# dluvizon/scene-aware-3d-multi-human

Hardware: AMD Instinct MI355X
Metric: optimizer iterations/sec (N humans x T frames) (higher is better)
Workload: dtype f32 (the two dense LBS contractions as split-16-bit MFMA operands -- three products of (hi, lo) fp16 / bf16 terms, fp32 accumulate; everything else plain fp32)

## Files before the change

include/mhmocap_hip.h:

```cpp
#ifndef MHMOCAP_HIP_H
#define MHMOCAP_HIP_H

#include <stddef.h>
#include <stdint.h>

#ifdef __cplusplus
extern "C" {
#endif

#define MH_NUM_JOINTS 24
#define MH_NUM_BETAS 10
#define MH_NUM_POSE_BASIS 207
#define MH_NUM_KP 17
#define MH_FEAT_STRIDE 224

typedef enum mh_status {
  MH_OK = 0,
  MH_ERR_INVALID = -1,
  MH_ERR_HIP = -2,
  MH_ERR_NO_DEVICE = -3,
  MH_ERR_UNSUPPORTED = -4
} mh_status;

typedef struct mh_model mh_model;
// ... 142 lines not shown
  const float* gbeta_b;
  const float* gxs_b;
  int B, NB, nbeta;
  long long off_betas;
  long long off_xscale;
} mh_person_sums;
int mh_rmsprop_step_person(float* params, float* grads, float* square_avg, float* momentum_buf, size_t n,
                           float lr, float alpha, float momentum, float eps, const float* log_src,
                           float* log_dst, int nlog, int32_t* poke_dst, int npoke, int32_t poke0,
                           int32_t poke1, const mh_person_sums* person, void* stream);
int mh_rmsprop_step_dev(float* params, const float* grads, float* square_avg, float* momentum_buf,
                        size_t n, float* lr_dev, float gamma, float alpha, float momentum, float eps,
                        void* stream);
int mh_adam_step(float* params, const float* grads, float* exp_avg, float* exp_avg_sq, size_t n,
                 int step, float lr, float beta1, float beta2, float eps, void* stream);

int mh_one_euro_scan(const float* x, float* y, int T, size_t E, float min_cutoff, float beta,
                     float frame_rate, void* stream);

int mh_one_euro_scan_shard(const float* x, float* y, int T, size_t E, float min_cutoff, float beta,
                           float frame_rate, int first_frame, float time_before,
                           const float* xprev_in, const float* dxprev_in, float* dxprev_out,
                           void* stream);

int mh_velocity_term(int T, int N, const float* pT , const float* prev_halo,
                     const float* next_halo, float coef, float* gpT, float* loss_out, void* stream);
size_t mh_filtered_verts_workspace_bytes(int T, size_t E);
int mh_filtered_verts_term(int T, size_t E, const float* verts, const float* verts_filt,
                           const float* prev_v, const float* prev_vf, const float* next_v,
                           const float* next_vf, float coef, float* gverts, float* loss_out,
                           void* ws, void* stream);
int mh_filtered_verts_term_init(int T, size_t E, const float* verts, const float* verts_filt,
                                const float* prev_v, const float* prev_vf, const float* next_v,
                                const float* next_vf, float coef, float* gverts, float* loss_out,
                                void* ws, void* stream);
int mh_filtered_verts_term_init_gated(int T, size_t E, const float* verts, const float* verts_filt,
                                      const float* prev_v, const float* prev_vf, const float* next_v,
                                      const float* next_vf, float coef, float* gverts, float* loss_out,
                                      const int32_t* live_dev, void* ws, void* stream);

int mh_pack_masks(const float* seg , int T, int N, int H, int W,
                  uint32_t* bits , float* area , void* stream);
int mh_erode_bits(const uint32_t* in, uint32_t* out , int T, int H, int W, void* stream);
int mh_stage_gates(const float* pose2d , const float* area , int B, float thr,
                   float min_area, float* pose2d_valid , float* mask_valid , void* stream);

// ... 272 lines not shown
```

scene-aware-3d-multi-human_amd/csrc/mh_optim.hip:

```cpp
#include "mh_common.h"

struct ProjP {
  int B, mode, has_kd;
  float K[9];
  float Kd[5];
  float jw[MH_NKP];
  float thr, w, h, coef;
  const float* joints;
  const float* pose2d;
  float* uv;
  float* gj;
  float* loss;
  int NB;
  const float* local;
  const float* xscale;
  const float* transl;
  float* gtransl;
};

__global__ __launch_bounds__(64) void k_project_loss(ProjP p) {
  const int b = blockIdx.x, j = threadIdx.x;
  float l = 0.f;
  float g3[3] = {0.f, 0.f, 0.f};
  if (j < MH_NKP) {
// ... 297 lines not shown
  return MH_OK;
}

__device__ __forceinline__ float one_euro_step(float xi, int i, float frame_rate, float min_cutoff, float beta, float& ti,
                                               float& tp, float& xp, float& dxp) {
#pragma clang fp contract(off)
  const float two_pi = 6.283185307179586f;
  ti = ti + (float)((double)i / (double)frame_rate);
  const float te = ti - tp;
  float r = two_pi * te;
  const float ad = r / (r + 1.f);
  const float dx = (xi - xp) / te;
  const float dxh = ad * dx + (1.f - ad) * dxp;
  const float cutoff = min_cutoff + beta * fabsf(dxh);
  r = (two_pi * cutoff) * te;
  const float a = r / (r + 1.f);
  const float xh = a * xi + (1.f - a) * xp;
  xp = xh;
  dxp = dxh;
  tp = ti;
  return xh;
}

__global__ void k_one_euro(const float* x, float* y, int T, size_t E, float min_cutoff, float beta, float frame_rate,
                           int i0, float t0, const float* xprev_in, const float* dxprev_in, float* dxprev_out) {
  for (size_t e = blockIdx.x * (size_t)blockDim.x + threadIdx.x; e < E; e += (size_t)gridDim.x * blockDim.x) {
    float xp, dxp, tp, ti;
    int first;
    if (xprev_in) {
      xp = xprev_in[e];
      dxp = dxprev_in[e];
      tp = ti = t0;
      first = 0;
    } else {
      xp = x[e];
      dxp = 0.f;
      tp = ti = 0.f;
      y[e] = xp;
      first = 1;
    }
    int k = first;
    for (; k + 8 <= T; k += 8) {
      float xv[8];
#pragma unroll
      for (int u = 0; u < 8; ++u) xv[u] = x[(size_t)(k + u) * E + e];
#pragma unroll
      for (int u = 0; u < 8; ++u)
        y[(size_t)(k + u) * E + e] = one_euro_step(xv[u], i0 + k + u, frame_rate, min_cutoff, beta, ti, tp, xp, dxp);
    }
    for (; k < T; ++k)
      y[(size_t)k * E + e] = one_euro_step(x[(size_t)k * E + e], i0 + k, frame_rate, min_cutoff, beta, ti, tp, xp, dxp);
    if (dxprev_out) dxprev_out[e] = dxp;
  }
}

static int one_euro_launch(const float* x, float* y, int T, size_t E, float min_cutoff, float beta, float frame_rate,
                           int i0, float t0, const float* xprev_in, const float* dxprev_in, float* dxprev_out,
                           void* stream) {
  MH_CHECK(x && y, "null argument");
  MH_CHECK(T >= 1 && E >= 1, "empty input");
  MH_CHECK((xprev_in == nullptr) == (dxprev_in == nullptr), "state arrays come in pairs");
  MH_CHECK(xprev_in || i0 == 0, "a shard that does not start the sequence needs the incoming state");
  const size_t nb = (E + 255) / 256;
  hipLaunchKernelGGL(k_one_euro, dim3((unsigned)(nb < 4096 ? nb : 4096)), dim3(256), 0, (hipStream_t)stream, x, y, T, E,
                     min_cutoff, beta, frame_rate, i0, t0, xprev_in, dxprev_in, dxprev_out);
  MH_LAUNCH_CHECK();
  return MH_OK;
}

extern "C" int mh_one_euro_scan(const float* x, float* y, int T, size_t E, float min_cutoff, float beta,
                                float frame_rate, void* stream) {
  return one_euro_launch(x, y, T, E, min_cutoff, beta, frame_rate, 0, 0.f, nullptr, nullptr, nullptr, stream);
}

extern "C" int mh_one_euro_scan_shard(const float* x, float* y, int T, size_t E, float min_cutoff, float beta,
                                      float frame_rate, int first_frame, float time_before, const float* xprev_in,
                                      const float* dxprev_in, float* dxprev_out, void* stream) {
  return one_euro_launch(x, y, T, E, min_cutoff, beta, frame_rate, first_frame, time_before, xprev_in, dxprev_in,
                         dxprev_out, stream);
}

__global__ __launch_bounds__(256) void k_velocity(int T, int N, const float* pT, const float* prev, const float* next,
                                                  float coef, float* gpT, float* loss_out) {
  __shared__ float s[256];
  const size_t E = (size_t)N * 3, n = (size_t)T * E;
  float acc = 0.f;
  for (size_t i = threadIdx.x; i < n; i += 256) {
    const size_t t = i / E, e = i % E;
    const float c = pT[i];
    float g = 0.f;
    if (t > 0 || prev) {
      const float d = c - (t > 0 ? pT[i - E] : prev[e]);
      acc += d * d;
      g += 2.f * d;
    }
// ... 246 lines not shown
```

scene-aware-3d-multi-human_amd/mhhip/_lib.py:

```python
import ctypes
import os
import re

import numpy as np

HERE = os.path.dirname(os.path.abspath(__file__))
LIB_PATH = os.environ.get('MHHIP_LIB') or os.path.join(HERE, 'libmhmocap_hip.so')
HEADER = os.path.join(os.path.dirname(os.path.dirname(HERE)), 'include', 'mhmocap_hip.h')

c_float_p = ctypes.POINTER(ctypes.c_float)
c_int_p = ctypes.POINTER(ctypes.c_int32)
vp = ctypes.c_void_p


class MhError(RuntimeError):
    pass


class ModelHost(ctypes.Structure):
    _fields_ = [('num_verts', ctypes.c_int32), ('num_faces', ctypes.c_int32),
                ('v_template', c_float_p), ('shapedirs', c_float_p), ('posedirs', c_float_p),
                ('J_regressor', c_float_p), ('lbs_weights', c_float_p), ('parents', c_int_p),
                ('faces', c_int_p), ('reg_alphapose', c_float_p), ('reg_h36m17', c_float_p),
                ('reg_mupots', c_float_p), ('reg_extra9', c_float_p)]
# ... 54 lines not shown
        L.mh_lbs_backward_ex.argtypes = [vp, ctypes.c_int, ctypes.c_int] + [vp] * 15
        L.mh_joints_regress_backward.argtypes = [vp, ctypes.c_int, ctypes.c_int, vp, ctypes.c_int, vp, vp, vp]
        L.mh_project_joints_loss.argtypes = [ctypes.c_int, vp, c_float_p, c_float_p, vp, ctypes.c_float, ctypes.c_int,
                                             ctypes.c_float, ctypes.c_float, ctypes.c_float, vp, vp, vp, vp]
        L.mh_project_joints_loss_w.argtypes = [ctypes.c_int, vp, c_float_p, c_float_p, c_float_p, vp, ctypes.c_float,
                                               ctypes.c_int, ctypes.c_float, ctypes.c_float, ctypes.c_float, vp, vp, vp, vp]
        L.mh_warmup_project_w.argtypes = [ctypes.c_int, ctypes.c_int, vp, vp, vp, c_float_p, c_float_p, c_float_p, vp,
                                          ctypes.c_float, ctypes.c_float, vp, vp, vp]
        L.mh_lbs_set_mode.argtypes = [ctypes.c_int]
        L.mh_lbs_set_forward_pipeline.argtypes = [ctypes.c_int]
        L.mh_rmsprop_step.argtypes = [vp, vp, vp, vp, ctypes.c_size_t] + [ctypes.c_float] * 4 + [vp]
        L.mh_rmsprop_step_log.argtypes = [vp, vp, vp, vp, ctypes.c_size_t] + [ctypes.c_float] * 4 + [vp, vp, ctypes.c_int, vp]
        L.mh_rmsprop_step_log_poke.argtypes = [vp, vp, vp, vp, ctypes.c_size_t] + [ctypes.c_float] * 4 + [vp, vp, ctypes.c_int, vp,
                                                                                                   ctypes.c_int, ctypes.c_int32, ctypes.c_int32, vp]
        L.mh_rmsprop_step_person.argtypes = [vp, vp, vp, vp, ctypes.c_size_t] + [ctypes.c_float] * 4 + [vp, vp, ctypes.c_int, vp,
                                                                                                 ctypes.c_int, ctypes.c_int32, ctypes.c_int32,
                                                                                                 ctypes.POINTER(PersonSums), vp]
        L.mh_lbs_backward_person_partials.argtypes = [vp, ctypes.c_int, vp, ctypes.POINTER(vp), ctypes.POINTER(vp)]
        L.mh_lbs_person_reduce.argtypes = [vp, ctypes.c_int, ctypes.c_int, vp, vp, vp, vp]
        L.mh_rmsprop_step_dev.argtypes = [vp, vp, vp, vp, ctypes.c_size_t, vp] + [ctypes.c_float] * 4 + [vp]
        L.mh_adam_step.argtypes = [vp, vp, vp, vp, ctypes.c_size_t, ctypes.c_int] + [ctypes.c_float] * 4 + [vp]
        L.mh_one_euro_scan.argtypes = [vp, vp, ctypes.c_int, ctypes.c_size_t] + [ctypes.c_float] * 3 + [vp]
        L.mh_one_euro_scan_shard.argtypes = [vp, vp, ctypes.c_int, ctypes.c_size_t] + [ctypes.c_float] * 3 + [ctypes.c_int, ctypes.c_float, vp, vp, vp, vp]
        L.mh_velocity_term.argtypes = [ctypes.c_int, ctypes.c_int, vp, vp, vp, ctypes.c_float, vp, vp, vp]
        L.mh_filtered_verts_term.argtypes = [ctypes.c_int, ctypes.c_size_t] + [vp] * 6 + [ctypes.c_float, vp, vp, vp, vp]
        L.mh_filtered_verts_term_init.argtypes = [ctypes.c_int, ctypes.c_size_t] + [vp] * 6 + [ctypes.c_float, vp, vp, vp, vp]
        L.mh_filtered_verts_term_init_gated.argtypes = [ctypes.c_int, ctypes.c_size_t] + [vp] * 6 + [ctypes.c_float, vp, vp, vp, vp, vp]
        L.mh_filtered_verts_workspace_bytes.restype = ctypes.c_size_t
        L.mh_filtered_verts_workspace_bytes.argtypes = [ctypes.c_int, ctypes.c_size_t]
        u32p = vp
        L.mh_warmup_project.argtypes = [ctypes.c_int, ctypes.c_int, vp, vp, vp, c_float_p, c_float_p, vp,
                                        ctypes.c_float, ctypes.c_float, vp, vp, vp]
        L.mh_pack_masks.argtypes = [vp] + [ctypes.c_int] * 4 + [u32p, vp, vp]
        L.mh_erode_bits.argtypes = [u32p, u32p] + [ctypes.c_int] * 3 + [vp]
        L.mh_stage_gates.argtypes = [vp, vp, ctypes.c_int, ctypes.c_float, ctypes.c_float, vp, vp, vp]
        L.mh_sil_mask_stats.argtypes = [u32p] + [ctypes.c_int] * 4 + [vp] * 8
        L.mh_sil_mask_stats_cached.argtypes = [u32p] + [ctypes.c_int] * 4 + [vp] * 9
        L.mh_prior_terms.argtypes = [ctypes.c_int] * 3 + [vp] * 6 + [ctypes.c_float] * 2 + [vp] * 6
        L.mh_reduce_sum.argtypes = [vp, ctypes.c_size_t, ctypes.c_float, vp, vp]
        L.mh_reduce_sum_multi.argtypes = [ctypes.c_int, ctypes.POINTER(vp), ctypes.POINTER(ctypes.c_size_t), ctypes.POINTER(vp), vp]
        L.mh_reduce_sum2.argtypes = [vp, vp, ctypes.c_size_t, ctypes.c_float, vp, vp, vp]
        L.mh_lowest_vertex.argtypes = [vp, ctypes.c_int, ctypes.c_int, vp, vp, vp]
        L.mh_contact_knn.argtypes = [vp, ctypes.c_int, vp, ctypes.c_int, ctypes.c_int, vp, vp]
        L.mh_scene_workspace_bytes.restype = ctypes.c_size_t
        L.mh_scene_workspace_bytes.argtypes = [ctypes.c_int] * 3
        L.mh_scene_median.argtypes = [ctypes.c_int] * 3 + [vp] * 8
# ... 140 lines not shown
```

scene-aware-3d-multi-human_amd/mhhip/engine.py:

```python
import ctypes
import pickle

import numpy as np
import torch

from . import _lib
from ._lib import check, ptr

H36M_ROW_ORDER = [6, 5, 4, 1, 2, 3, 16, 15, 14, 11, 12, 13, 8, 10, 0, 7, 9]
REG_ALPHAPOSE, REG_H36M17, REG_MUPOTS, REG_EXTRA9 = 0, 1, 2, 3
NUM_REG_JOINTS = {0: 17, 1: 17, 2: 17, 3: 9}


class _ChStub(object):

    def __setstate__(self, state):
        self.__dict__.update(state if isinstance(state, dict) else {'x': state})

    def __array__(self, dtype=None, copy=None):
        x = self.__dict__.get('x', None)
        if x is None:
            raise ValueError('unsupported chumpy object in the SMPL pickle')
        return np.array(x, dtype=dtype) if copy else np.asarray(x, dtype=dtype)

# ... 275 lines not shown
    check(_lib.lib().mh_rmsprop_step_log_poke(ptr(params), ptr(grads), ptr(sq), ptr(buf), params.numel(), lr, alpha, momentum,
                                              eps, ptr(log_src), ptr(log_dst), nlog, poke_dst.data_ptr(), min(len(poke) - 1, 2),
                                              poke[0], poke[1], _lib.stream_ptr(params.device)))


def adam_step(params, grads, m, v, step, lr, b1=0.5, b2=0.5, eps=1e-6):
    check(_lib.lib().mh_adam_step(ptr(params), ptr(grads), ptr(m), ptr(v), params.numel(), int(step), lr, b1, b2, eps,
                                  _lib.stream_ptr(params.device)))


def one_euro_scan(x, min_cutoff, beta, frame_rate=25.0, out=None):
    x = x.contiguous()
    if out is None:
        y = torch.empty_like(x)
    else:
        assert out.is_contiguous() and out.dtype == x.dtype and out.numel() == x.numel() and out.device == x.device
        y = out.view(x.shape)
    T = x.shape[0]
    check(_lib.lib().mh_one_euro_scan(ptr(x), ptr(y), T, x.numel() // T, float(min_cutoff), float(beta),
                                      float(frame_rate), _lib.stream_ptr(x.device)))
    return y


def one_euro_time_before(first_frame, frame_rate=25.0):
    t = np.float32(0)
    for i in range(1, int(first_frame)):
        t = np.float32(t + np.float32(i / frame_rate))
    return float(t)


def one_euro_scan_shard(x, min_cutoff, beta, first_frame, state_in=None, frame_rate=25.0):
    x = x.contiguous()
    y = torch.empty_like(x)
    T = x.shape[0]
    E = x.numel() // T
    dx_out = torch.empty(E, dtype=torch.float32, device=x.device)
    xp, dxp = (None, None) if state_in is None else state_in
    check(_lib.lib().mh_one_euro_scan_shard(ptr(x), ptr(y), T, E, float(min_cutoff), float(beta), float(frame_rate),
                                            int(first_frame), one_euro_time_before(first_frame, frame_rate),
                                            ptr(xp), ptr(dxp), ptr(dx_out), _lib.stream_ptr(x.device)))
    return y, (y[-1].reshape(-1).contiguous(), dx_out)


def velocity_term(pT, coef, gpT, prev_halo=None, next_halo=None):
    T, N = pT.shape[0], pT.shape[1]
    loss = torch.empty(1, dtype=torch.float32, device=pT.device)
# ... 17 lines not shown
```

scene-aware-3d-multi-human_amd/mhhip/sequence.py:

```python
import ctypes

import numpy as np
import os
import torch

from . import _lib, engine, queues
from ._lib import check, ptr

LOG_KEYS = ['loss_pose24j', 'loss_depth', 'loss_silhouette', 'reg_ref_poses', 'reg_scale', 'reg_contact',
            'reg_foot_sliding', 'reg_vel', 'reg_filter_verts']
COEF_KEYS = ['proj2d', 'depth', 'silhouette', 'reg_velocity', 'reg_verts_filter', 'reg_poses', 'reg_scales',
             'reg_contact', 'reg_foot_sliding']
PEN_DEFAULTS = dict(reg_scene_pen=0.0, scene_pen_margin=0.05, scene_pen_band=0.5, scene_pen_edge=0.25)
PEN_LOG = 12
ORDER_DEFAULTS = dict(reg_order=0.0, order_margin=0.05, order_delta=0.5)
ORDER_LOG = 13


_SHARED_STREAMS = {}


def _shared_stream(device, role):
    key = (torch.device(device).index or 0, role)
    st = _SHARED_STREAMS.get(key)
# ... 59 lines not shown
        self.ws2 = model.backward_workspace(B)
        self.kp_ws = torch.empty(max(1, _lib.lib().mh_keypoint_workspace_bytes(model.handle, B)), dtype=torch.uint8, device=self.dev)
        self.fv_ws = torch.empty(_lib.lib().mh_filtered_verts_workspace_bytes(T, N * self.V * 3), dtype=torch.uint8, device=self.dev)
        self.verts = z(B, self.V, 3)
        self.vposed = z(B, self.V, 3)
        self.gverts = None
        self.kp = z(B, 17, 3)
        self.gj = z(B, 17, 3)
        self.uv = z(B, 17, 2)
        self.loss2d = z(B)
        self.prior_body = z(B)
        self.loss3 = z(3)
        self.vel_loss = z(1)
        self.filt_loss = z(1)
        self.log = z(max_cycles, 16)
        self.tmp_log = self._grads_log[n:]
        self._log_pending = None
        self.scene_pts = None
        self.scene_grid = None
        self.scene_M = 0
        self.scene_zmap = None
        self._scene_dev = None
        self._scene_pending = False
        self.verts_filt = None
        self.pT_filt = None
        self.has_images = False
        self.halo = None
        self.phase = torch.zeros(4, dtype=torch.int32, device=self.dev)
        self._phase_const = [torch.tensor([1, k], dtype=torch.int32, device=self.dev) for k in (0, 1)]
        self._phase_host = [0, 0, 0]
        self._phase_poke = None
        self._filt_gate = False
        self.batch_frames = None
        self.timing = None
        if self._pen:
            self.pen_body = z(B)
            self.pen_acc = torch.zeros(B, dtype=torch.int64, device=self.dev)
        if self._order:
            self.order_body = z(B)
            self.order_acc = torch.zeros(B, 3, dtype=torch.int64, device=self.dev)
            self.order_gate = None

    def enable_timing(self, on=True):
        self.timing = {} if on else None

    def _tic(self, name):
        if self.timing is None:
            return None
# ... 20 lines not shown
    def set_batch_table(self, table):
        if table is None:
            self.batch_frames = None
            return
        n = self.nbatches * self.batch
        if getattr(self, 'batch_frames', None) is None or self.batch_frames.numel() != n:
            self.batch_frames = torch.full((n,), -1, dtype=torch.int32, device=self.dev)
        if isinstance(table, torch.Tensor):
            self.batch_frames.copy_(table.reshape(-1), non_blocking=True)
        else:
            self.batch_frames.copy_(torch.as_tensor(np.ascontiguousarray(table, dtype=np.int32).reshape(-1)))

    def _view(self, buf, i, shape):
        return buf[int(self.offs[i]):int(self.offs[i + 1])].view(*shape)

    def leaf(self, name, buf=None):
        buf = self.params if buf is None else buf
        T, N = self.T, self.N
        i, shape = {'poses_T': (0, (T, N, 3)), 'poses_smpl': (1, (T, N, 72)), 'zmin_lin': (2, (T,)),
                    'zmax_lin': (3, (T,)), 'betas': (4, (N, 10)), 'xscale': (5, (N,))}[name]
        return self._view(buf, i, shape)

    def set_leaves(self, poses_T, poses_smpl, betas, zmin_lin, zmax_lin, xscale=None):
        self.leaf('poses_T').copy_(_dev(poses_T, self.dev).view(self.T, self.N, 3))
        self.leaf('poses_smpl').copy_(_dev(poses_smpl, self.dev).view(self.T, self.N, 72))
        self.leaf('betas').copy_(_dev(betas, self.dev).view(self.N, 10))
        self.leaf('zmin_lin').copy_(_dev(zmin_lin, self.dev).view(self.T))
        self.leaf('zmax_lin').copy_(_dev(zmax_lin, self.dev).view(self.T))
        if xscale is not None:
            self.leaf('xscale').copy_(_dev(xscale, self.dev).view(self.N))
        else:
            self.leaf('xscale').zero_()
        self.sq.zero_()
        self.buf.zero_()

    def stage(self, pose2d, poses_ref, valid, betas_ref, seg_mask=None, depths=None):
        T, N, H, W = self.T, self.N, self.H, self.W
        L = _lib.lib()
        st = _lib.stream_ptr(self.dev)
        if getattr(self, '_graphs', None):
            torch.cuda.current_stream(self.dev).synchronize()
            self._graphs = {}
            self._lane_tests = {}
            self._pickers = {}
        self._scene_dev = None
        self.pose2d = _dev(pose2d, self.dev).view(self.B, 17, 3)
# ... 194 lines not shown
        k = d['ready']
        s = d['sets'][k]
        d['front'], d['ready'] = s, None
        self._phase_poke = (1, k)
        self.scene_pts = s['pts']
        self.scene_grid = s['grid']
        self.scene_M = self.H * self.W
        self._scene_event = s['ev']
        self._scene_pending = True

    def _scene_sel(self):
        d = self._scene_dev
        if d is None or os.environ.get('MHHIP_UNIFORM') == '0':
            return None
        if self.scene_pts is None or any(self.scene_pts is x['pts'] for x in d['sets']):
            return d['sets']
        return None

    def _flush_phase(self):
        if self._phase_poke is not None:
            (live, k), self._phase_poke = self._phase_poke, None
            self.phase[1:3].copy_(self._phase_const[k])
            self._phase_host[1], self._phase_host[2] = live, k

    def enable_filter_gate(self):
        if self.verts_filt is not None or self.pT_filt is not None:
            return self._filt_gate
        self.pT_filt = torch.zeros(self.T, self.N, 3, dtype=torch.float32, device=self.dev)
        self.verts_filt = torch.zeros(self.T, self.N, self.V, 3, dtype=torch.float32, device=self.dev)
        self._filt_gate = True
        return True

    def _filters_live(self):
        if self._filt_gate and not self._phase_host[0]:
            self.phase[0:1].fill_(1)
            self._phase_host[0] = 1

    def main_stream(self):
        return torch.cuda.current_stream(self.dev)

    def stream_ctx(self, stream):
        return torch.cuda.stream(stream)

    def scene_median_rows(self, depths_t, back_t, zmin, zmax, med, msk, stream):
        rows, frames = depths_t.shape
        check(_lib.lib().mh_scene_median_t(frames, 1, rows, ptr(depths_t), ptr(back_t), ptr(zmin), ptr(zmax), ptr(med), ptr(msk),
                                           ptr(self._scene_dev['ws']), stream.cuda_stream))

    def scene_fill_plane(self, val, mask, ksize, stream):
        check(_lib.lib().mh_scene_fill(self.H, self.W, int(ksize), 1, ptr(val), ptr(mask), ptr(self._scene_dev['ws']), stream.cuda_stream))

    def scene_device_image(self, images):
# ... 60 lines not shown
        if regress:
            self._regress(_lib.stream_ptr(self.dev))

    def _regress(self, st):
        check(_lib.lib().mh_joints_regress(self.m.handle, self.joints_reg[0], self.B, ptr(self.verts),
                                           ptr(self.leaf('poses_T')), self.joints_reg[1], ptr(self.kp), st))

    def _halo_forward(self, h, st):
        Bh = int(h['poses'].shape[0])
        if getattr(self, '_halo_verts', None) is None or self._halo_verts.shape[0] != Bh:
            self._halo_verts = torch.empty(Bh, self.V, 3, dtype=torch.float32, device=self.dev)
            self._halo_ws = self.m.workspace(Bh)
        check(_lib.lib().mh_lbs_forward(self.m.handle, Bh, self.N, ptr(self.leaf('betas')), ptr(h['poses']), ptr(self.leaf('xscale')),
                                        ptr(h['transl']), ptr(self._halo_verts), None, None, ptr(self._halo_ws), st))
        k = 0
        h['v_prev'] = h['v_next'] = None
        if h.get('has_prev'):
            h['v_prev'] = self._halo_verts[:self.N]
            k = self.N
        if h.get('has_next'):
            h['v_next'] = self._halo_verts[k:k + self.N]

    def step_local(self, lr, alpha=0.5, momentum=0.9, eps=1e-8):
        self._wait_scene_snapshot()
        self._flush_person()
        self._flush_log()
        self._flush_phase()
        lo = self.shared_lo
        engine.rmsprop_step(self.params[:lo], self.grads[:lo], self.sq[:lo], self.buf[:lo], float(lr), alpha, momentum, eps)

    def step_shared(self, lr, alpha=0.5, momentum=0.9, eps=1e-8):
        lo = self.shared_lo
        engine.rmsprop_step(self.params[lo:], self.grads[lo:], self.sq[lo:], self.buf[lo:], float(lr), alpha, momentum, eps)

    def keypoint_terms(self, st):
        jwp = None if self.joint_w is None else self.joint_w.ctypes.data_as(_lib.c_float_p)
        Kp = self.K.ctypes.data_as(_lib.c_float_p)
        Kdp = None if self.Kd is None else self.Kd.ctypes.data_as(_lib.c_float_p)
        check(_lib.lib().mh_keypoint_terms(self.m.handle, self.B, ptr(self.leaf('poses_T')), Kp, Kdp, jwp, ptr(self.pose2d), self.thr,
                                           float(self.W), float(self.H), float(self.c['proj2d']), ptr(self.kp), ptr(self.uv),
                                           ptr(self.gj), ptr(self.loss2d), ptr(self.ws), ptr(self.ws2), ptr(self.kp_ws), st))
        self._kp_chunk = True

    def _side_stream(self):
        if not hasattr(self, '_side'):
            self._side = _shared_stream(self.dev, 'side')
        return self._side

    def cycle(self, row, use_images=True, raster=None):
        self._flush_person()
        nj = raster is not None and use_images and self.has_images
        self.cycle_begin(join=not nj, raster=raster if (use_images and self.has_images) else None)
        self.cycle_finish(row, use_images, raster)

    def cycle_begin(self, join=True, raster=None):
        self._flush_log()
        if not torch.cuda.is_current_stream_capturing():
            self._flush_phase()
        clear_in_fwd = (not join) and raster is not None and _lib.lib().mh_lbs_get_mode() != 0
        if not clear_in_fwd:
            self._grads_log.zero_()
        main = torch.cuda.current_stream(self.dev)
        side = self._side_stream()
        side.wait_stream(main)
        self.forward(regress=False, raster=raster, clear=self._grads_log if clear_in_fwd else None)
        self._leaf_terms_later = not join
        if join:
            self._leaf_terms(side.cuda_stream)
            main.wait_stream(side)

    def _leaf_terms(self, st):
        L, c = _lib.lib(), self.c
        T, N = self.T, self.N
        g, log = self.grads, self.tmp_log
        pT = self.leaf('poses_T')
        h = self.halo or {}
        if self.has_images:
            check(L.mh_sil_mask_stats_cached(ptr(self.bits), T, N, self.H, self.W, ptr(pT), ptr(self.p2d_valid),
                                             ptr(self.mask_valid), ptr(self.front), ptr(self.sil_apply), ptr(self.sil_D),
                                             ptr(self.sil_S), ptr(self.sil_tag), st))
# ... 9 lines not shown
            self.keypoint_terms(st)
            return
        jwp = None if self.joint_w is None else self.joint_w.ctypes.data_as(_lib.c_float_p)
        Kp = self.K.ctypes.data_as(_lib.c_float_p)
        Kdp = None if self.Kd is None else self.Kd.ctypes.data_as(_lib.c_float_p)
        self._kp_chunk = False
        self._regress(st)
        check(_lib.lib().mh_project_joints_loss_w(self.B, ptr(self.kp), Kp, Kdp, jwp, ptr(self.pose2d), self.thr, 0, float(self.W),
                                                  float(self.H), float(self.c['proj2d']), ptr(self.uv), ptr(self.gj), ptr(self.loss2d), st))

    def cycle_finish(self, row, use_images=True, raster=None, scene_ready=False):
        self._finish_a(use_images, raster, scene_ready=scene_ready)
        self._finish_b(row, use_images, raster)

    def _finish_a(self, use_images=True, raster=None, scene_ready=False):
        L = _lib.lib()
        main = torch.cuda.current_stream(self.dev)
        st = main.cuda_stream
        c = self.c
        T, N, B = self.T, self.N, self.B
        h = self.halo or {}
        sel = self._scene_sel() if scene_ready else None
        scene = self.scene_pts is not None or sel is not None
        filt = self.verts_filt is not None and self.pT_filt is not None
        images = use_images and self.has_images
        if self._pen and self.halo is not None:
            raise ValueError('the scene-penetration term (reg_scene_pen != 0) is not available in a frame-sharded run')
        if self._order and self.halo is not None:
            raise ValueError('the depth-ordering term (reg_order != 0) is not available in a frame-sharded run')
        need_gv = scene or filt or (images and raster is not None) or not self.kp_fused
        log = self.tmp_log
        gv = None
        if need_gv:
            if self.gverts is None:
                self.gverts = torch.empty_like(self.verts)
            gv = self.gverts
        self._gv_cur = gv
        side = self._side_stream()
        side.wait_stream(main)
        s2 = side.cuda_stream

        def side_branch():
            self._regress_project(s2)
            if self._leaf_terms_later:
                self._leaf_terms_later = False
                self._leaf_terms(s2)
            with torch.cuda.stream(side):
                if need_gv and filt and h.get('poses') is not None:
                    self._halo_forward(h, s2)
                if need_gv:
                    if filt:
                        E = N * self.V * 3
                        ev = self._tic('filtered_verts')
                        if self._filt_gate:
                            check(L.mh_filtered_verts_term_init_gated(T, E, ptr(self.verts), ptr(self.verts_filt), ptr(h.get('v_prev')),
                                                                      ptr(h.get('vf_prev')), ptr(h.get('v_next')), ptr(h.get('vf_next')),
                                                                      float(c['reg_verts_filter']), ptr(gv), ptr(log[8:9]),
                                                                      self.phase.data_ptr(), ptr(self.fv_ws), s2))
                        else:
                            check(L.mh_filtered_verts_term_init(T, E, ptr(self.verts), ptr(self.verts_filt), ptr(h.get('v_prev')),
                                                                ptr(h.get('vf_prev')), ptr(h.get('v_next')), ptr(h.get('vf_next')),
                                                                float(c['reg_verts_filter']), ptr(gv), ptr(log[8:9]), ptr(self.fv_ws), s2))
                        self._toc(ev)
                    else:
                        gv.zero_()
                if not self.kp_fused:
                    check(L.mh_joints_regress_backward(self.m.handle, self.joints_reg[0], B, ptr(self.gj), self.joints_reg[1], ptr(gv),
                                                       ptr(self.leaf('poses_T', self.grads)), s2))
                if not hasattr(self, '_ev_gv'):
                    self._ev_gv = torch.cuda.Event()
                self._ev_gv.record(side)
            self._scene_done = False
            sums = [(self.loss2d, log[0:1]), (self.prior_body, log[3:4])]
            if scene and (self._scene_dev is None or scene_ready):
                sums += self._scene_terms(s2, reduce=False, sel=sel)
                self._scene_done = True
            _lib.reduce_sum_multi(sums, s2)
        joined = False
        main_first = images and raster is not None
        if not main_first:
            side_branch()
        if images:
            if raster is not None:
# ... 87 lines not shown
        zmap = self._pen_zmap()
        if zmap is None:
            return False
        check(L.mh_scene_pen_term(self.B, self.V, self.H, self.W, Kp, ptr(self.verts), ptr(zmap), *tail))
        return True

    def _order_term(self, raster, st):
        if not self._order:
            return
        c, log = self.c, self.tmp_log
        check(_lib.lib().mh_order_term(*raster.dims, ptr(raster.ws), ptr(self.bits), ptr(self.ebits), ptr(self.order_gate),
                                       float(c['reg_order']), float(c['order_margin']), float(c['order_delta']),
                                       ptr(self.leaf('poses_T', self.grads)), ptr(self.order_body), None, None, ptr(self.order_acc), st))
        _lib.reduce_sum_multi([(self.order_body, log[ORDER_LOG:ORDER_LOG + 1])], st)

    def _finish_b(self, row, use_images=True, raster=None):
        L = _lib.lib()
        st = _lib.stream_ptr(self.dev)
        T, N, B = self.T, self.N, self.B
        g = self.grads
        gpT, gposes = self.leaf('poses_T', g), self.leaf('poses_smpl', g)
        gbetas, gxs = self.leaf('betas', g), self.leaf('xscale', g)
        pT = self.leaf('poses_T')
        filt = self.verts_filt is not None and self.pT_filt is not None
        gv, log = self._gv_cur, self.tmp_log
        if self.scene_pts is not None and not self._scene_done:
            ev = self._tic('scene_terms')
            if self._scene_pending:
                torch.cuda.current_stream(self.dev).wait_event(self._scene_event)
                self._scene_pending = False
            self._scene_terms(st)
            self._toc(ev)
        ev = self._tic('lbs_backward')
        fin, self._raster_fin = getattr(self, '_raster_fin', None), None
        if getattr(self, '_kp_chunk', False):
            pb, px = (None, None) if self._person_now else (ptr(gbetas), ptr(gxs))
            args = (self.m.handle, B, N, ptr(self.leaf('betas')), ptr(self.leaf('poses_smpl')), ptr(self.vposed),
                    ptr(gv), ptr(gposes), ptr(gpT), pb, px, ptr(self.ws), ptr(self.ws2),
                    ctypes.byref(fin) if fin is not None else None, st)
            check(L.mh_lbs_backward_kp_fin(*args))
        else:
            check(L.mh_lbs_backward(self.m.handle, B, N, ptr(self.leaf('betas')), ptr(self.leaf('poses_smpl')),
                                    ptr(self.leaf('xscale')), ptr(pT), ptr(self.vposed), ptr(gv), ptr(self.gj) if self.kp_fused else None, ptr(gposes),
                                    ptr(gpT), None if self._person_now else ptr(gbetas), None if self._person_now else ptr(gxs),
                                    ptr(self.ws), ptr(self.ws2), st))
        self._toc(ev)
        if row is not None:
            self.log[row].copy_(log)

    def step(self, lr, alpha=0.5, momentum=0.9, eps=1e-8):
        self._wait_scene_snapshot()
        poke, self._phase_poke = self._phase_poke, None
        person = None
        if self._person_pending:
            self._person_pending = False
            person = self._person_sums()
        if self._log_pending is not None or poke is not None or person is not None:
            row, self._log_pending = self._log_pending, None
            engine.rmsprop_step_log(self.params, self.grads, self.sq, self.buf, float(lr), self.tmp_log if row is not None else None,
                                    self.log[row] if row is not None else None, alpha, momentum, eps,
                                    poke_dst=self.phase[1:3] if poke is not None else None, poke=poke, person=person)
            if poke is not None:
                self._phase_host[1], self._phase_host[2] = poke
        else:
            engine.rmsprop_step(self.params, self.grads, self.sq, self.buf, float(lr), alpha, momentum, eps)

    def _person_sums(self):
        gb, gx = ctypes.c_void_p(), ctypes.c_void_p()
        check(_lib.lib().mh_lbs_backward_person_partials(self.m.handle, self.B, ptr(self.ws2), ctypes.byref(gb), ctypes.byref(gx)))
        return _lib.PersonSums(gb.value, gx.value, self.B, self.N, 10, int(self.offs[4]), -1 if self.freeze_xscale else int(self.offs[5]))

    def _flush_person(self):
        if self._person_pending:
            self._person_pending = False
            g = self.grads
            check(_lib.lib().mh_lbs_person_reduce(self.m.handle, self.B, self.N, ptr(self.ws2), ptr(self.leaf('betas', g)),
                                                  ptr(self.leaf('xscale', g)), _lib.stream_ptr(self.dev)))

    def _flush_log(self):
        if self._log_pending is not None:
            row, self._log_pending = self._log_pending, None
            self.log[row].copy_(self.tmp_log)

    def _graph_key(self, raster):
        scene = None
        sel = self._scene_sel()
        if sel is not None:
            scene = ('sel', sel[0]['grid'].data_ptr(), sel[1]['grid'].data_ptr())
        elif self.scene_pts is not None:
            scene = (self.scene_pts.data_ptr(), self.scene_grid.data_ptr(), self.scene_M)
        rast = None if raster is None else (raster.ws.data_ptr(), raster.faces.data_ptr())
        bt = None if getattr(self, 'batch_frames', None) is None else self.batch_frames.data_ptr()
        L = _lib.lib()
        glob = (L.mh_raster_get_deterministic(), L.mh_raster_get_sort_margin(), L.mh_lbs_get_mode(), L.mh_raster_get_path(),
                L.mh_raster_get_winners(), float(L.mh_raster_get_sort_defer()), L.mh_lbs_get_forward_pipeline()) if raster is not None else None
        pen = None
        if self._pen:
            zm = tuple(x['zmap'].data_ptr() for x in sel) if sel is not None else (None if self._pen_zmap() is None else self._pen_zmap().data_ptr())
            pen = (float(self.c['reg_scene_pen']), float(self.c['scene_pen_margin']), float(self.c['scene_pen_band']),
                   float(self.c['scene_pen_edge']), zm)
        hk = None if self.halo is None else (bool(self.halo.get('has_prev')), bool(self.halo.get('has_next')), self.halo.get('poses') is not None)
        key = (rast, scene, self.verts_filt is not None and self.pT_filt is not None, self._filt_gate, hk, bt, glob)
        if pen is not None:
            key = key + (pen,)
        if self._order:
            key = key + (('order', float(self.c['reg_order']), float(self.c['order_margin']), float(self.c['order_delta'])),)
        return key

    def raster_terms(self, znear=1.0, zfar=100.0):
        if getattr(self, '_raster', None) is None:
            from . import raster as _raster
            self._raster = _raster.RasterTerms(self, znear, zfar)
        return self._raster

    def replay(self, key, fn, wait_scene=True):
        if wait_scene and self._scene_pending:
            torch.cuda.current_stream(self.dev).wait_event(self._scene_event)
            self._scene_pending = False
        if not hasattr(self, '_graphs'):
            self._graphs = {}
        if not hasattr(self, '_lane_tests'):
            self._lane_tests = {}
        g = self._graphs.get(key)
        if g is None:
            fn()
# ... 7 lines not shown
            lt = self._lane_tests.get(key) if want else None
            if lt is None and want and key not in self._lane_tests:
                lt = self._lane_tests[key] = queues.LaneTest(queues.plan(self.dev), torch.cuda.current_stream(self.dev).cuda_stream)
                lt.clean = True
            if lt is not None and not lt.done and not getattr(lt, 'recorded', False):
                if self._scene_dev.get('snap_pending') or self._scene_pending:
                    lt.clean = False
                main = torch.cuda.current_stream(self.dev)
                lt.before(main)
                g.replay()
                lt.after(main)
            else:
                if lt is not None and not lt.done and lt.poll() and lt.choice is not None:
                    self._scene_move(queues.plan(self.dev).view(lt.choice))
                g.replay()

    def cycle_graphed(self, row, raster=None, scene_update=False):
        self._flush_person()
        self._person_now = bool(self.defer_person) and os.environ.get('MHHIP_DEFER_PERSON') != '0'
        try:
            key = self._graph_key(raster) + (self._person_now,)
            self._flush_log()
            self._flush_phase()
            if scene_update and queues.enabled():
                self._scene_pick(key)
            if scene_update:
                self.scene_device_mark()
            scene_ready = self._scene_dev is not None

            def body():
                nj = raster is not None and self.has_images
                self.cycle_begin(join=not nj, raster=raster if self.has_images else None)
                self.cycle_finish(None, raster=raster, scene_ready=scene_ready)
            self.replay(('full+scene' if scene_ready else 'full',) + key, body)
            if scene_update:
                self.scene_device_launch()
            self._log_pending = row
            self._person_pending = self._person_now
        finally:
            self._person_now = False

    def step_dev(self, alpha=0.5, momentum=0.9, eps=1e-8, gamma=0.99, lr0=0.01):
        if not hasattr(self, 'lr_dev'):
            self.lr_dev = torch.full((1,), lr0, dtype=torch.float32, device=self.dev)
        self._flush_person()
        self._flush_log()
        self._flush_phase()
        self._wait_scene_snapshot()
        check(_lib.lib().mh_rmsprop_step_dev(ptr(self.params), ptr(self.grads), ptr(self.sq), ptr(self.buf),
                                             self.params.numel(), ptr(self.lr_dev), gamma, alpha, momentum, eps,
                                             _lib.stream_ptr(self.dev)))

    def set_filters(self, pT_filt, verts_filt):
        verts_filt = verts_filt.view(self.T, self.N, self.V, 3)
        if self.pT_filt is None or self.pT_filt.shape != pT_filt.shape:
            self.pT_filt = pT_filt.clone()
        else:
            self.pT_filt.copy_(pT_filt)
        if self.verts_filt is None or self.verts_filt.shape != verts_filt.shape:
            self.verts_filt = verts_filt.clone()
        else:
            self.verts_filt.copy_(verts_filt)
        self._filters_live()

    def update_filters(self, c1=0.01, b1=0.02, c2=0.001, b2=0.5):
        pT = self.leaf('poses_T')
        if self.pT_filt is not None and self.verts_filt is not None and self.pT_filt.numel() == pT.numel():
            engine.one_euro_scan(pT, c1, b1, out=self.pT_filt)
            self.forward(regress=False)
            engine.one_euro_scan(self.verts.view(self.T, -1), c2, b2, out=self.verts_filt)
            self._filters_live()
            return
        pf = engine.one_euro_scan(pT, c1, b1)
        self.forward(regress=False)
        self.set_filters(pf, engine.one_euro_scan(self.verts.view(self.T, -1), c2, b2))

    def one_euro_shard(self, x, min_cutoff, beta, first_frame, state_in=None):
        return engine.one_euro_scan_shard(x, min_cutoff, beta, first_frame, state_in)

    def read_log(self, rows, nbatches_total=None):
        self._flush_log()
        raw = self.log[:rows].cpu().numpy().astype(np.float64)
        nb = float(nbatches_total or self.nbatches)
        out = []
        for r in raw:
            d = {'loss_pose24j': r[0] / nb, 'loss_depth': r[1] / nb, 'loss_silhouette': r[2] / nb,
                 'reg_ref_poses': (r[3] + r[9]) / nb, 'reg_scale': r[10] + r[11], 'reg_contact': r[5] / nb,
                 'reg_foot_sliding': r[6] / nb, 'reg_vel': r[7], 'reg_filter_verts': r[8]}
            if self._pen:
                d['reg_scene_pen'] = r[PEN_LOG]
            if self._order:
                d['reg_order'] = r[ORDER_LOG]
            out.append({k: np.float32(v) for k, v in d.items()})
# ... 2 lines not shown
```

scene-aware-3d-multi-human_amd/mhmocap/optimizer.py:

```python
import os

import numpy as np
import torch
import torch.distributed as dist

from mhhip import _lib, engine
from mhhip.sequence import SequenceEngine, COEF_KEYS
from .smpl import SMPL
from .transforms import get_focal, softplus_np

try:
    from tqdm import tqdm
except Exception:
    tqdm = None


def frames_arg(frames, T):
    idx = np.arange(T) if frames is None else np.asarray(frames).reshape(-1)
    if idx.size == 0 or not np.issubdtype(idx.dtype, np.integer) or idx.min() < 0 or idx.max() >= T:
        raise ValueError('frames must be indices in [0, %d), got %r' % (T, frames))
    return idx.astype(np.int64)


class SMPLOptimizerBase(object):
# ... 471 lines not shown
        lr = 0.01
        e.sq.zero_()
        e.buf.zero_()
        sh.leaves_changed()
        sh.refresh_halo()
        if (self.use_graphs and world == 1 and os.environ.get('MHHIP_UNIFORM') != '0' and hasattr(e, 'enable_filter_gate')):
            if (num_iter > 30 and scene_mode == 'device' and e.has_images and self._backmasks is not None and e._scene_dev is None):
                sh.scene_setup(self._backmasks)
            if any(c % update_filters_every == 0 for c in range(30, num_iter)):
                e.enable_filter_gate()
        deferring = bool(self.use_graphs and world == 1 and hasattr(e, 'defer_person'))
        if deferring:
            defer_before = e.defer_person
            e.defer_person, e.freeze_xscale = True, not self.optim_scale_factor
        cycles = range(num_iter)
        if verbose and tqdm is not None and rank == 0:
            cycles = tqdm(cycles)
        for cycle in cycles:
            if cycle >= 30 and cycle % update_filters_every == 0:
                if world > 1:
                    sh.update_filters(min_cutoff1, beta1, min_cutoff2, beta2)
                else:
                    e.update_filters(min_cutoff1, beta1, min_cutoff2, beta2)
                self.poses_T_filtered = e.pT_filt.view(e.T, self.num_people, 1, 3)
                self.verts_filtered = e.verts_filt
            if tables is not None:
                e.set_batch_table(tables[cycle])
            scene_now = cycle >= 30 and e.has_images and self._backmasks is not None
            dev_scene = scene_now and scene_mode == 'device'
            if dev_scene and e._scene_dev is None:
                sh.scene_setup(self._backmasks)
            if world > 1:
                if dev_scene:
                    sh.scene_update()
                sh.cycle(cycle, raster=raster, graphs=self.use_graphs)
            else:
                sh.cycle(cycle, raster=raster, graphs=self.use_graphs, scene_update=dev_scene)
            if dev_scene:
                e.scene_device_swap()
            if not self.optim_scale_factor:
                e.leaf('xscale', e.grads).zero_()
            sh.step(lr)
            lr *= 0.99
            if check_every and cycle % check_every == 0:
                self.check_replicas()
        if deferring:
            e._flush_person()
            e.defer_person = defer_before
# ... 227 lines not shown
```

Before: 1638.

## Defer one-euro filter update into captured cycle via device-gated fused scan kernel

Instead of running the two one-euro scans and an extra forward pass eagerly whenever the filters are refreshed, the update is recorded as pending. Inside the next cycle it runs as a single gated kernel that filters both vertices and root translations, reusing the vertices the cycle's forward pass just produced. A device control word arms the gate and is cleared afterwards through the optimizer-step poke, so the captured graph stays the same. This removes an extra forward pass and several launches per filter update, at the cost of more complex host state and flush points.

```diff
diff --git a/include/mhmocap_hip.h b/include/mhmocap_hip.h
--- a/include/mhmocap_hip.h
+++ b/include/mhmocap_hip.h
@@ -188,6 +188,9 @@
                            float frame_rate, int first_frame, float time_before,
                            const float* xprev_in, const float* dxprev_in, float* dxprev_out,
                            void* stream);
+
+int mh_one_euro_scan2_gated(const int32_t* ctl, const float* xa, float* ya, size_t Ea, const float* xb,
+                            float* yb, size_t Eb, int T, float frame_rate, void* stream);
 
 int mh_velocity_term(int T, int N, const float* pT , const float* prev_halo,
                      const float* next_halo, float coef, float* gpT, float* loss_out, void* stream);
diff --git a/scene-aware-3d-multi-human_amd/csrc/mh_optim.hip b/scene-aware-3d-multi-human_amd/csrc/mh_optim.hip
--- a/scene-aware-3d-multi-human_amd/csrc/mh_optim.hip
+++ b/scene-aware-3d-multi-human_amd/csrc/mh_optim.hip
@@ -343,9 +343,10 @@
   return xh;
 }
 
-__global__ void k_one_euro(const float* x, float* y, int T, size_t E, float min_cutoff, float beta, float frame_rate,
-                           int i0, float t0, const float* xprev_in, const float* dxprev_in, float* dxprev_out) {
-  for (size_t e = blockIdx.x * (size_t)blockDim.x + threadIdx.x; e < E; e += (size_t)gridDim.x * blockDim.x) {
+__device__ __forceinline__ void one_euro_channels(const float* x, float* y, int T, size_t E, float min_cutoff, float beta,
+                                                  float frame_rate, int i0, float t0, const float* xprev_in,
+                                                  const float* dxprev_in, float* dxprev_out, size_t e0, size_t stride) {
+  for (size_t e = e0; e < E; e += stride) {
     float xp, dxp, tp, ti;
     int first;
     if (xprev_in) {
@@ -375,6 +376,24 @@
   }
 }
 
+__global__ void k_one_euro(const float* x, float* y, int T, size_t E, float min_cutoff, float beta, float frame_rate,
+                           int i0, float t0, const float* xprev_in, const float* dxprev_in, float* dxprev_out) {
+  one_euro_channels(x, y, T, E, min_cutoff, beta, frame_rate, i0, t0, xprev_in, dxprev_in, dxprev_out,
+                    blockIdx.x * (size_t)blockDim.x + threadIdx.x, (size_t)gridDim.x * blockDim.x);
+}
+
+__global__ void k_one_euro2_gated(const int* ctl, const float* xa, float* ya, size_t Ea, unsigned nba, const float* xb,
+                                  float* yb, size_t Eb, int T, float frame_rate) {
+  if (ctl[0] == 0) return;
+  const float* par = (const float*)(ctl + 1);
+  if (blockIdx.x < nba)
+    one_euro_channels(xa, ya, T, Ea, par[0], par[1], frame_rate, 0, 0.f, nullptr, nullptr, nullptr,
+                      blockIdx.x * (size_t)blockDim.x + threadIdx.x, (size_t)nba * blockDim.x);
+  else
+    one_euro_channels(xb, yb, T, Eb, par[2], par[3], frame_rate, 0, 0.f, nullptr, nullptr, nullptr,
+                      (blockIdx.x - nba) * (size_t)blockDim.x + threadIdx.x, (size_t)(gridDim.x - nba) * blockDim.x);
+}
+
 static int one_euro_launch(const float* x, float* y, int T, size_t E, float min_cutoff, float beta, float frame_rate,
                            int i0, float t0, const float* xprev_in, const float* dxprev_in, float* dxprev_out,
                            void* stream) {
@@ -392,6 +411,18 @@
 extern "C" int mh_one_euro_scan(const float* x, float* y, int T, size_t E, float min_cutoff, float beta,
                                 float frame_rate, void* stream) {
   return one_euro_launch(x, y, T, E, min_cutoff, beta, frame_rate, 0, 0.f, nullptr, nullptr, nullptr, stream);
+}
+
+extern "C" int mh_one_euro_scan2_gated(const int32_t* ctl, const float* xa, float* ya, size_t Ea, const float* xb, float* yb,
+                                       size_t Eb, int T, float frame_rate, void* stream) {
+  MH_CHECK(ctl && xa && ya && xb && yb, "null argument");
+  MH_CHECK(T >= 1 && Ea >= 1 && Eb >= 1, "empty input");
+  const size_t na = (Ea + 255) / 256, nb = (Eb + 255) / 256;
+  const unsigned nba = (unsigned)(na < 4096 ? na : 4096), nbb = (unsigned)(nb < 4096 ? nb : 4096);
+  hipLaunchKernelGGL(k_one_euro2_gated, dim3(nba + nbb), dim3(256), 0, (hipStream_t)stream, (const int*)ctl, xa, ya, Ea, nba,
+                     xb, yb, Eb, T, frame_rate);
+  MH_LAUNCH_CHECK();
+  return MH_OK;
 }
 
 extern "C" int mh_one_euro_scan_shard(const float* x, float* y, int T, size_t E, float min_cutoff, float beta,
diff --git a/scene-aware-3d-multi-human_amd/mhhip/_lib.py b/scene-aware-3d-multi-human_amd/mhhip/_lib.py
--- a/scene-aware-3d-multi-human_amd/mhhip/_lib.py
+++ b/scene-aware-3d-multi-human_amd/mhhip/_lib.py
@@ -100,6 +100,7 @@
         L.mh_adam_step.argtypes = [vp, vp, vp, vp, ctypes.c_size_t, ctypes.c_int] + [ctypes.c_float] * 4 + [vp]
         L.mh_one_euro_scan.argtypes = [vp, vp, ctypes.c_int, ctypes.c_size_t] + [ctypes.c_float] * 3 + [vp]
         L.mh_one_euro_scan_shard.argtypes = [vp, vp, ctypes.c_int, ctypes.c_size_t] + [ctypes.c_float] * 3 + [ctypes.c_int, ctypes.c_float, vp, vp, vp, vp]
+        L.mh_one_euro_scan2_gated.argtypes = [vp, vp, vp, ctypes.c_size_t, vp, vp, ctypes.c_size_t, ctypes.c_int, ctypes.c_float, vp]
         L.mh_velocity_term.argtypes = [ctypes.c_int, ctypes.c_int, vp, vp, vp, ctypes.c_float, vp, vp, vp]
         L.mh_filtered_verts_term.argtypes = [ctypes.c_int, ctypes.c_size_t] + [vp] * 6 + [ctypes.c_float, vp, vp, vp, vp]
         L.mh_filtered_verts_term_init.argtypes = [ctypes.c_int, ctypes.c_size_t] + [vp] * 6 + [ctypes.c_float, vp, vp, vp, vp]
diff --git a/scene-aware-3d-multi-human_amd/mhhip/engine.py b/scene-aware-3d-multi-human_amd/mhhip/engine.py
--- a/scene-aware-3d-multi-human_amd/mhhip/engine.py
+++ b/scene-aware-3d-multi-human_amd/mhhip/engine.py
@@ -321,6 +321,21 @@
     return y
 
 
+def one_euro_ctl(armed, ca, ba, cb, bb, device):
+    words = np.array([ca, ba, cb, bb], np.float32).view(np.int32)
+    return torch.tensor([int(bool(armed))] + words.tolist(), dtype=torch.int32, device=device)
+
+
+def one_euro_scan2_gated(ctl, xa, ya, xb, yb, frame_rate=25.0, stream=None):
+    T = xa.shape[0]
+    for x, y in ((xa, ya), (xb, yb)):
+        assert x.is_contiguous() and y.is_contiguous() and x.dtype == y.dtype == torch.float32
+        assert x.shape[0] == T and y.numel() == x.numel() and x.device == y.device == ctl.device
+    assert ctl.dtype == torch.int32 and ctl.numel() >= 5 and ctl.is_contiguous()
+    check(_lib.lib().mh_one_euro_scan2_gated(ptr(ctl), ptr(xa), ptr(ya), xa.numel() // T, ptr(xb), ptr(yb), xb.numel() // T, T,
+                                             float(frame_rate), _lib.stream_ptr(xa.device) if stream is None else stream))
+
+
 def one_euro_time_before(first_frame, frame_rate=25.0):
     t = np.float32(0)
     for i in range(1, int(first_frame)):
diff --git a/scene-aware-3d-multi-human_amd/mhhip/sequence.py b/scene-aware-3d-multi-human_amd/mhhip/sequence.py
--- a/scene-aware-3d-multi-human_amd/mhhip/sequence.py
+++ b/scene-aware-3d-multi-human_amd/mhhip/sequence.py
@@ -105,8 +105,12 @@
         self.scene_zmap = None
         self._scene_dev = None
         self._scene_pending = False
-        self.verts_filt = None
-        self.pT_filt = None
+        self._verts_filt = None
+        self._pT_filt = None
+        self._oe_ctl = None
+        self._oe_arm_src = {}
+        self._oe_pending = None
+        self._oe_armed = 0
         self.has_images = False
         self.halo = None
         self.phase = torch.zeros(4, dtype=torch.int32, device=self.dev)
@@ -173,6 +177,7 @@
         return self._view(buf, i, shape)
 
     def set_leaves(self, poses_T, poses_smpl, betas, zmin_lin, zmax_lin, xscale=None):
+        self._flush_filters()
         self.leaf('poses_T').copy_(_dev(poses_T, self.dev).view(self.T, self.N, 3))
         self.leaf('poses_smpl').copy_(_dev(poses_smpl, self.dev).view(self.T, self.N, 72))
         self.leaf('betas').copy_(_dev(betas, self.dev).view(self.N, 10))
@@ -413,12 +418,70 @@
             (live, k), self._phase_poke = self._phase_poke, None
             self.phase[1:3].copy_(self._phase_const[k])
             self._phase_host[1], self._phase_host[2] = live, k
+        if self._oe_armed == 2:
+            self._oe_ctl[0:1].zero_()
+            self._oe_armed = 0
+
+    @property
+    def verts_filt(self):
+        self._flush_filters()
+        return self._verts_filt
+
+    @verts_filt.setter
+    def verts_filt(self, v):
+        self._flush_filters()
+        self._verts_filt = v
+
+    @property
+    def pT_filt(self):
+        self._flush_filters()
+        return self._pT_filt
+
+    @pT_filt.setter
+    def pT_filt(self, v):
+        self._flush_filters()
+        self._pT_filt = v
+
+    def filter_buffers(self):
+        return self._pT_filt, self._verts_filt
+
+    def _flush_filters(self):
+        if self._oe_pending is None or torch.cuda.is_current_stream_capturing():
+            return
+        (c1, b1, c2, b2), self._oe_pending = self._oe_pending, None
+        engine.one_euro_scan(self.leaf('poses_T'), c1, b1, out=self._pT_filt)
+        self.forward(regress=False)
+        engine.one_euro_scan(self.verts.view(self.T, -1), c2, b2, out=self._verts_filt)
+
+    def _arm_filters(self):
+        if self._oe_pending is not None and (self.halo is not None or self._verts_filt is None or self._pT_filt is None):
+            self._flush_filters()
+        if self._oe_pending is not None:
+            par, self._oe_pending = self._oe_pending, None
+            src = self._oe_arm_src.get(par)
+            if src is None:
+                c1, b1, c2, b2 = par
+                src = self._oe_arm_src[par] = engine.one_euro_ctl(1, c2, b2, c1, b1, device=self.dev)
+            self._oe_words().copy_(src)
+            self._oe_armed = 1
+        elif self._oe_armed == 2:
+            self._oe_ctl[0:1].zero_()
+            self._oe_armed = 0
+
+    def _oe_words(self):
+        if self._oe_ctl is None:
+            self._oe_ctl = engine.one_euro_ctl(0, 0.0, 0.0, 0.0, 0.0, device=self.dev)
+        return self._oe_ctl
+
+    def _oe_scan(self, st):
+        engine.one_euro_scan2_gated(self._oe_words(), self.verts.view(self.T, -1), self._verts_filt.view(self.T, -1),
+                                    self.leaf('poses_T'), self._pT_filt, stream=st)
 
     def enable_filter_gate(self):
-        if self.verts_filt is not None or self.pT_filt is not None:
+        if self._verts_filt is not None or self._pT_filt is not None:
             return self._filt_gate
-        self.pT_filt = torch.zeros(self.T, self.N, 3, dtype=torch.float32, device=self.dev)
-        self.verts_filt = torch.zeros(self.T, self.N, self.V, 3, dtype=torch.float32, device=self.dev)
+        self._pT_filt = torch.zeros(self.T, self.N, 3, dtype=torch.float32, device=self.dev)
+        self._verts_filt = torch.zeros(self.T, self.N, self.V, 3, dtype=torch.float32, device=self.dev)
         self._filt_gate = True
         return True
 
@@ -525,6 +588,7 @@
             h['v_next'] = self._halo_verts[k:k + self.N]
 
     def step_local(self, lr, alpha=0.5, momentum=0.9, eps=1e-8):
+        self._flush_filters()
         self._wait_scene_snapshot()
         self._flush_person()
         self._flush_log()
@@ -533,6 +597,7 @@
         engine.rmsprop_step(self.params[:lo], self.grads[:lo], self.sq[:lo], self.buf[:lo], float(lr), alpha, momentum, eps)
 
     def step_shared(self, lr, alpha=0.5, momentum=0.9, eps=1e-8):
+        self._flush_filters()
         lo = self.shared_lo
         engine.rmsprop_step(self.params[lo:], self.grads[lo:], self.sq[lo:], self.buf[lo:], float(lr), alpha, momentum, eps)
 
@@ -552,13 +617,16 @@
 
     def cycle(self, row, use_images=True, raster=None):
         self._flush_person()
+        self._arm_filters()
         nj = raster is not None and use_images and self.has_images
         self.cycle_begin(join=not nj, raster=raster if (use_images and self.has_images) else None)
         self.cycle_finish(row, use_images, raster)
+        self._oe_armed = 2 if self._oe_armed else 0
 
     def cycle_begin(self, join=True, raster=None):
         self._flush_log()
         if not torch.cuda.is_current_stream_capturing():
+            self._flush_filters()
             self._flush_phase()
         clear_in_fwd = (not join) and raster is not None and _lib.lib().mh_lbs_get_mode() != 0
         if not clear_in_fwd:
@@ -614,7 +682,7 @@
         h = self.halo or {}
         sel = self._scene_sel() if scene_ready else None
         scene = self.scene_pts is not None or sel is not None
-        filt = self.verts_filt is not None and self.pT_filt is not None
+        filt = self._verts_filt is not None and self._pT_filt is not None
         images = use_images and self.has_images
         if self._pen and self.halo is not None:
             raise ValueError('the scene-penetration term (reg_scene_pen != 0) is not available in a frame-sharded run')
@@ -643,14 +711,16 @@
                 if need_gv:
                     if filt:
                         E = N * self.V * 3
+                        if self.halo is None and self._pT_filt.numel() == T * N * 3:
+                            self._oe_scan(s2)
                         ev = self._tic('filtered_verts')
                         if self._filt_gate:
-                            check(L.mh_filtered_verts_term_init_gated(T, E, ptr(self.verts), ptr(self.verts_filt), ptr(h.get('v_prev')),
+                            check(L.mh_filtered_verts_term_init_gated(T, E, ptr(self.verts), ptr(self._verts_filt), ptr(h.get('v_prev')),
                                                                       ptr(h.get('vf_prev')), ptr(h.get('v_next')), ptr(h.get('vf_next')),
                                                                       float(c['reg_verts_filter']), ptr(gv), ptr(log[8:9]),
                                                                       self.phase.data_ptr(), ptr(self.fv_ws), s2))
                         else:
-                            check(L.mh_filtered_verts_term_init(T, E, ptr(self.verts), ptr(self.verts_filt), ptr(h.get('v_prev')),
+                            check(L.mh_filtered_verts_term_init(T, E, ptr(self.verts), ptr(self._verts_filt), ptr(h.get('v_prev')),
                                                                 ptr(h.get('vf_prev')), ptr(h.get('v_next')), ptr(h.get('vf_next')),
                                                                 float(c['reg_verts_filter']), ptr(gv), ptr(log[8:9]), ptr(self.fv_ws), s2))
                         self._toc(ev)
@@ -784,7 +854,7 @@
         gpT, gposes = self.leaf('poses_T', g), self.leaf('poses_smpl', g)
         gbetas, gxs = self.leaf('betas', g), self.leaf('xscale', g)
         pT = self.leaf('poses_T')
-        filt = self.verts_filt is not None and self.pT_filt is not None
+        filt = self._verts_filt is not None and self._pT_filt is not None
         gv, log = self._gv_cur, self.tmp_log
         if self.scene_pts is not None and not self._scene_done:
             ev = self._tic('scene_terms')
@@ -811,8 +881,16 @@
             self.log[row].copy_(log)
 
     def step(self, lr, alpha=0.5, momentum=0.9, eps=1e-8):
+        self._flush_filters()
         self._wait_scene_snapshot()
         poke, self._phase_poke = self._phase_poke, None
+        poke_dst = self.phase[1:3]
+        if self._oe_armed == 2:
+            if poke is None:
+                poke, poke_dst = (0,), self._oe_ctl[0:1]
+            else:
+                self._oe_ctl[0:1].zero_()
+            self._oe_armed = 0
         person = None
         if self._person_pending:
             self._person_pending = False
@@ -821,8 +899,8 @@
             row, self._log_pending = self._log_pending, None
             engine.rmsprop_step_log(self.params, self.grads, self.sq, self.buf, float(lr), self.tmp_log if row is not None else None,
                                     self.log[row] if row is not None else None, alpha, momentum, eps,
-                                    poke_dst=self.phase[1:3] if poke is not None else None, poke=poke, person=person)
-            if poke is not None:
+                                    poke_dst=poke_dst if poke is not None else None, poke=poke, person=person)
+            if poke is not None and len(poke) == 2:
                 self._phase_host[1], self._phase_host[2] = poke
         else:
             engine.rmsprop_step(self.params, self.grads, self.sq, self.buf, float(lr), alpha, momentum, eps)
@@ -862,7 +940,7 @@
             pen = (float(self.c['reg_scene_pen']), float(self.c['scene_pen_margin']), float(self.c['scene_pen_band']),
                    float(self.c['scene_pen_edge']), zm)
         hk = None if self.halo is None else (bool(self.halo.get('has_prev')), bool(self.halo.get('has_next')), self.halo.get('poses') is not None)
-        key = (rast, scene, self.verts_filt is not None and self.pT_filt is not None, self._filt_gate, hk, bt, glob)
+        key = (rast, scene, self._verts_filt is not None and self._pT_filt is not None, self._filt_gate, hk, bt, glob)
         if pen is not None:
             key = key + (pen,)
         if self._order:
@@ -916,6 +994,7 @@
             key = self._graph_key(raster) + (self._person_now,)
             self._flush_log()
             self._flush_phase()
+            self._arm_filters()
             if scene_update and queues.enabled():
                 self._scene_pick(key)
             if scene_update:
@@ -927,6 +1006,7 @@
                 self.cycle_begin(join=not nj, raster=raster if self.has_images else None)
                 self.cycle_finish(None, raster=raster, scene_ready=scene_ready)
             self.replay(('full+scene' if scene_ready else 'full',) + key, body)
+            self._oe_armed = 2 if self._oe_armed else 0
             if scene_update:
                 self.scene_device_launch()
             self._log_pending = row
@@ -937,6 +1017,7 @@
     def step_dev(self, alpha=0.5, momentum=0.9, eps=1e-8, gamma=0.99, lr0=0.01):
         if not hasattr(self, 'lr_dev'):
             self.lr_dev = torch.full((1,), lr0, dtype=torch.float32, device=self.dev)
+        self._flush_filters()
         self._flush_person()
         self._flush_log()
         self._flush_phase()
@@ -946,23 +1027,31 @@
                                              _lib.stream_ptr(self.dev)))
 
     def set_filters(self, pT_filt, verts_filt):
+        self._flush_filters()
         verts_filt = verts_filt.view(self.T, self.N, self.V, 3)
-        if self.pT_filt is None or self.pT_filt.shape != pT_filt.shape:
-            self.pT_filt = pT_filt.clone()
-        else:
-            self.pT_filt.copy_(pT_filt)
-        if self.verts_filt is None or self.verts_filt.shape != verts_filt.shape:
-            self.verts_filt = verts_filt.clone()
-        else:
-            self.verts_filt.copy_(verts_filt)
+        if self._pT_filt is None or self._pT_filt.shape != pT_filt.shape:
+            self._pT_filt = pT_filt.clone()
+        else:
+            self._pT_filt.copy_(pT_filt)
+        if self._verts_filt is None or self._verts_filt.shape != verts_filt.shape:
+            self._verts_filt = verts_filt.clone()
+        else:
+            self._verts_filt.copy_(verts_filt)
         self._filters_live()
 
     def update_filters(self, c1=0.01, b1=0.02, c2=0.001, b2=0.5):
+        self._flush_filters()
         pT = self.leaf('poses_T')
-        if self.pT_filt is not None and self.verts_filt is not None and self.pT_filt.numel() == pT.numel():
-            engine.one_euro_scan(pT, c1, b1, out=self.pT_filt)
+        live = self._phase_host[0] or not self._filt_gate
+        if self._pT_filt is not None and self._verts_filt is not None and self._pT_filt.numel() == pT.numel() and live:
+            self._oe_pending = (float(c1), float(b1), float(c2), float(b2))
+            if self.halo is not None:
+                self._flush_filters()
+            return
+        if self._pT_filt is not None and self._verts_filt is not None and self._pT_filt.numel() == pT.numel():
+            engine.one_euro_scan(pT, c1, b1, out=self._pT_filt)
             self.forward(regress=False)
-            engine.one_euro_scan(self.verts.view(self.T, -1), c2, b2, out=self.verts_filt)
+            engine.one_euro_scan(self.verts.view(self.T, -1), c2, b2, out=self._verts_filt)
             self._filters_live()
             return
         pf = engine.one_euro_scan(pT, c1, b1)
diff --git a/scene-aware-3d-multi-human_amd/mhmocap/optimizer.py b/scene-aware-3d-multi-human_amd/mhmocap/optimizer.py
--- a/scene-aware-3d-multi-human_amd/mhmocap/optimizer.py
+++ b/scene-aware-3d-multi-human_amd/mhmocap/optimizer.py
@@ -517,8 +517,9 @@
                     sh.update_filters(min_cutoff1, beta1, min_cutoff2, beta2)
                 else:
                     e.update_filters(min_cutoff1, beta1, min_cutoff2, beta2)
-                self.poses_T_filtered = e.pT_filt.view(e.T, self.num_people, 1, 3)
-                self.verts_filtered = e.verts_filt
+                pf, vf = e.filter_buffers() if hasattr(e, 'filter_buffers') else (e.pT_filt, e.verts_filt)
+                self.poses_T_filtered = pf.view(e.T, self.num_people, 1, 3)
+                self.verts_filtered = vf
             if tables is not None:
                 e.set_batch_table(tables[cycle])
             scene_now = cycle >= 30 and e.has_images and self._backmasks is not None
```

Measured after the change: 1657 (median of 4 runs). No clear change (+1.2%).
